# uberkk/ImageCompressionLearnedLiftingandLearnedTreeBasedModels

Hardware: AMD Instinct MI355X
Metric: Mpixels/sec (lifting DWT + entropy-model fwd) at 512x512 RGB (higher is better)
Workload: dtype f32 storage, f16x3 arithmetic (3 fp16 MFMA products per fp32 MAC, fp32 accumulate)

## Files before the change

### imagecompressionlearnedliftingandlearnedtreebasedmodels_amd/csrc/conv_f16x3.hip

```cpp
#include "common.h"
#include "split_f16.h"
#include "lifting_f16.h"
#include <string.h>
#include <type_traits>

namespace lldwt {

constexpr int F3_CK = 32;
constexpr int F3_TH = 8, F3_TW = 32;
constexpr int F3_IH = F3_TH + 2, F3_IW = F3_TW + 2, F3_NPX = F3_IH * F3_IW;
constexpr int F3_PITCH = F3_CK * 2 + 16;
constexpr int F3_PART = F3_NPX * F3_PITCH;
constexpr int F3_BUF = 2 * F3_PART;
constexpr int F3_LDS = 2 * F3_BUF + 64;
constexpr int F3_OCB = 128;
constexpr int F3_STEP_BYTES = 2048;
constexpr int F3_CHUNK_BYTES = 9 * 2 * F3_STEP_BYTES;
constexpr int F3_HDR = 256;
constexpr int F3_NTASK = F3_NPX * (F3_CK / 8);
constexpr int F3_R = (F3_NTASK + 255) / 256;

constexpr int F1_HDR = 2048;
constexpr int F1_CHUNK_BYTES = 2 * F3_STEP_BYTES;
constexpr int F1_NBLK = (F3_NPX + 31) / 32;
// ... 538 lines not shown
                if (u == 22) F3_FUSED_BLOCK(0, sdst)
                if (u == 26) F3_FUSED_BLOCK(1, sdst)
                if (u == 30) F3_FUSED_BLOCK(2, sdst)
            } else {
                if (u < F3_R) F3_TASK_LOAD(u, c1)
                if (u >= 24) F3_TASK_STORE((u - 24) >> 1, (u - 24) & 1, c1, sdst)
            }
            const half8 A_h = ah[st % 6], A_l = al[st % 6];
#pragma unroll
            for (int n = 0; n < 4; ++n) {
                if constexpr (PREC == 0) {
                    acc[hf * 4 + n] = mma32<0>(A_l, bh[u & 1][n], acc[hf * 4 + n]);
                    if constexpr (!IN16) acc[hf * 4 + n] = mma32<0>(A_h, bl[u & 1][n], acc[hf * 4 + n]);
                }
                acc[hf * 4 + n] = mma32<PREC>(A_h, bh[u & 1][n], acc[hf * 4 + n]);
            }
#pragma unroll
            for (int i = 0; i < (PREC == 0 ? 12 : 4); ++i) {
                __builtin_amdgcn_sched_group_barrier(0x008, 1, 0);
                __builtin_amdgcn_sched_group_barrier(0x100, 1, 0);
                __builtin_amdgcn_sched_group_barrier(0x020, 1, 0);
                __builtin_amdgcn_sched_group_barrier(0x002, PREC == 0 ? 4 : 10, 0);
                __builtin_amdgcn_sched_group_barrier(0x200, 1, 0);
            }
            __builtin_amdgcn_sched_barrier(0);
        }
#undef F3_BLOAD
        __syncthreads();
    }
    }
#undef F3_TASK_LOAD
#undef F3_TASK_STORE
#undef F3_FUSED_BLOCK
#undef F3_FUSED_LOAD

    F3_STAMP(10)
    if constexpr (S16) {
        const int px = lane & 15;
        const int ocw = ocb * F3_OCB + __builtin_amdgcn_readfirstlane(wave) * 32;
        const int och = 4 * (lane >> 4);
        float* ybase = a.y + (z * a.cout + ocw) * hw + (int64_t)y0 * w;
        const unsigned loff = (unsigned)och * (unsigned)hw + (unsigned)(x0 + px);
        const bool full = y0 + F3_TH <= h && x0 + F3_TW <= w;
        const float slope = a.act == LLDWT_ACT_LRELU ? 0.01f : (a.act == LLDWT_ACT_RELU ? 0.f : 1.f);
#pragma unroll
        for (int hv = 0; hv < 2; ++hv) {
#pragma unroll
            for (int q = 0; q < 4; ++q) {
                const int oc = ocw + 16 * hv + och + q;
                if (oc < a.cout) {
                    const float bq = a.bias ? a.bias[plane * a.cout + oc] : 0.f;
                    float* yq = ybase + (int64_t)(16 * hv + q) * hw;
                    if (full && a.act != LLDWT_ACT_TANH) {
#pragma unroll
                        for (int n = 0; n < 16; ++n) {
                            const float v = acc16[hv][n][q] * out_scale + bq;
                            yq[(n >> 1) * w + 16 * (n & 1) + loff] = fmaxf(v, v * slope);
                        }
                    } else {
#pragma unroll
                        for (int n = 0; n < 16; ++n)
                            if (y0 + (n >> 1) < h && x0 + 16 * (n & 1) + px < w)
                                yq[(n >> 1) * w + 16 * (n & 1) + loff] = act_apply(acc16[hv][n][q] * out_scale + bq, a.act);
                    }
                }
            }
        }
    } else {
        const int gx = x0 + (lane & 31);
        const int ocw = ocb * F3_OCB + __builtin_amdgcn_readfirstlane(wave) * 32;
        const int och = 4 * (lane >> 5);
        float* ybase = a.y + (z * a.cout + ocw) * hw + (int64_t)y0 * w;
        const unsigned loff = (unsigned)och * (unsigned)hw + (unsigned)gx;
        float bq[16];
#pragma unroll
        for (int q = 0; q < 16; ++q) {
            const int oc = ocw + (q & 3) + 8 * (q >> 2) + och;
            bq[q] = a.bias ? a.bias[plane * a.cout + (oc < a.cout ? oc : a.cout - 1)] : 0.f;
        }
#pragma unroll
        for (int q = 0; q < 16; ++q) asm volatile("" ::"v"(bq[q]));
        const bool full = y0 + F3_TH <= h && x0 + F3_TW <= w;
        if (full && a.act != LLDWT_ACT_TANH) {
            const float slope = a.act == LLDWT_ACT_LRELU ? 0.01f : (a.act == LLDWT_ACT_RELU ? 0.f : 1.f);
#pragma unroll
            for (int q = 0; q < 16; ++q) {
                if (ocw + (q & 3) + 8 * (q >> 2) + och < a.cout) {
                    float* yq = ybase + (int64_t)((q & 3) + 8 * (q >> 2)) * hw;
#pragma unroll
                    for (int n = 0; n < 8; ++n) {
                        const float v = acc[n][q] * out_scale + bq[q];
                        yq[n * w + loff] = fmaxf(v, v * slope);
                    }
                }
            }
        } else if (full) {
#pragma unroll
            for (int q = 0; q < 16; ++q) {
                if (ocw + (q & 3) + 8 * (q >> 2) + och < a.cout) {
                    float* yq = ybase + (int64_t)((q & 3) + 8 * (q >> 2)) * hw;
#pragma unroll
                    for (int n = 0; n < 8; ++n) yq[n * w + loff] = fast_tanh(acc[n][q] * out_scale + bq[q]);
                }
            }
        } else {
#pragma unroll
            for (int q = 0; q < 16; ++q) {
                if (ocw + (q & 3) + 8 * (q >> 2) + och < a.cout) {
                    float* yq = ybase + (int64_t)((q & 3) + 8 * (q >> 2)) * hw;
#pragma unroll
                    for (int n = 0; n < 8; ++n)
                        if (y0 + n < h && gx < w) yq[n * w + loff] = act_apply(acc[n][q] * out_scale + bq[q], a.act);
                }
            }
        }
    }
    F3_STAMP(11)
    F3_STAMP(15)
}

constexpr int W3_NE = F3_IH * 4 * 16;
constexpr int W3_PART = W3_NE * 32;
constexpr int W3_BUF = 2 * W3_PART;
constexpr int W3_DUMP = 2 * W3_BUF;
constexpr int W3_COLP = 144;
constexpr int W3_COL = W3_DUMP + 64;
constexpr int W3_PP = W3_COL + 2 * F3_IH * 17 * W3_COLP;
constexpr int W3_BIAS = W3_PP + 1536;
constexpr int W3_LDS = W3_BIAS + F3_OCB * 4;
constexpr int W3_LDS_EARLIER = W3_BIAS;
constexpr int W3_RING = 6;
static_assert(12 % W3_RING == 0 && W3_RING <= 6, "weight ring");
static_assert(W3_PP % 16 == 0 && F1_PP * 4 <= 1536, "LDS layout");

__device__ __forceinline__ void w3_row_mma(f4_t (&t)[4], const h8_t& wh, const h8_t& wl, const h8_t (&ch)[4], const h8_t (&cl)[4]) {
    asm volatile(
        "v_mfma_f32_16x16x32_f16 %0, %4, %6, 0\n\t"
        "v_mfma_f32_16x16x32_f16 %1, %4, %7, 0\n\t"
        "v_mfma_f32_16x16x32_f16 %2, %4, %8, 0\n\t"
        "v_mfma_f32_16x16x32_f16 %3, %4, %9, 0\n\t"
        "v_mfma_f32_16x16x32_f16 %0, %5, %10, %0\n\t"
        "v_mfma_f32_16x16x32_f16 %1, %5, %11, %1\n\t"
        "v_mfma_f32_16x16x32_f16 %2, %5, %12, %2\n\t"
        "v_mfma_f32_16x16x32_f16 %3, %5, %13, %3\n\t"
        "v_mfma_f32_16x16x32_f16 %0, %5, %6, %0\n\t"
        "v_mfma_f32_16x16x32_f16 %1, %5, %7, %1\n\t"
        "v_mfma_f32_16x16x32_f16 %2, %5, %8, %2\n\t"
        "v_mfma_f32_16x16x32_f16 %3, %5, %9, %3\n\t"
        "s_nop 7\n\ts_nop 7\n\ts_nop 4"
        : "=&v"(t[0]), "=&v"(t[1]), "=&v"(t[2]), "=&v"(t[3])
        : "v"(wl), "v"(wh), "v"(ch[0]), "v"(ch[1]), "v"(ch[2]), "v"(ch[3]), "v"(cl[0]), "v"(cl[1]), "v"(cl[2]), "v"(cl[3]));
}

__device__ __forceinline__ void wino_u(const float* g, double (&u)[4]) {
    const double g0 = g[0], g1 = g[1], g2 = g[2];
    u[0] = g0; u[1] = (g0 + g1 + g2) * 0.5; u[2] = (g0 - g1 + g2) * 0.5; u[3] = g2;
}

__global__ void k_f3w_umax(const float* __restrict__ w, int64_t nrows, uint8_t* __restrict__ packed, int64_t plane_bytes, int64_t woff) {
    const int plane = blockIdx.y;
    float m = 0.f;
    for (int64_t i = blockIdx.x * (int64_t)blockDim.x + threadIdx.x; i < nrows; i += (int64_t)gridDim.x * blockDim.x) {
        double u[4];
        wino_u(w + ((int64_t)plane * nrows + i) * 3, u);
        for (int k = 0; k < 4; ++k) m = fmaxf(m, fabsf((float)u[k]));
    }
#pragma unroll
    for (int o = 32; o > 0; o >>= 1) m = fmaxf(m, __shfl_down(m, o, 64));
    float* hdr = reinterpret_cast<float*>(packed + (int64_t)plane * plane_bytes + woff);
    if ((threadIdx.x & 63) == 0 && m > 0.f) atomicMax(reinterpret_cast<int*>(hdr + 1), __float_as_int(m));
}

__global__ void k_f3w_pack(const float* __restrict__ w, uint8_t* __restrict__ packed, int cin, int cout, int64_t plane_bytes, int64_t woff) {
    const int plane = blockIdx.y;
    uint8_t* pp = packed + (int64_t)plane * plane_bytes + woff;
    float* hdr = reinterpret_cast<float*>(pp);
    const double su = pow2_scale<15>(hdr[1]);
    const int nch = w3_nch(cin), nocb = (cout + F3_OCB - 1) / F3_OCB;
    const int64_t n = (int64_t)nocb * 4 * nch * W3_NST * 64 * 8;
    const float* wp = w + (int64_t)plane * cout * cin * 9;
    _Float16* out = reinterpret_cast<_Float16*>(pp + F3_HDR);
    for (int64_t i = blockIdx.x * (int64_t)blockDim.x + threadIdx.x; i < n; i += (int64_t)gridDim.x * blockDim.x) {
        int64_t r = i;
        const int j = (int)(r % 8); r /= 8;
        const int lane = (int)(r % 64); r /= 64;
        const int st = (int)(r % W3_NST); r /= W3_NST;
        const int chunk = (int)(r % nch); r /= nch;
        const int wv = (int)(r % 4); r /= 4;
        const int ocb = (int)r;
        const int oc = ocb * F3_OCB + wv * 32 + (lane & 31), ic = chunk * W3_CK + 8 * (lane >> 5) + j;
        const int dy = st >> 2, xi = st & 3;
        float v = 0.f;
        if (oc < cout && ic < cin) {
            double u[4];
            wino_u(wp + ((int64_t)oc * cin + ic) * 9 + dy * 3, u);
            v = (float)(u[xi] * su);
        }
        const _Float16 hi = (_Float16)v;
        const int64_t step = ((int64_t)(ocb * 4 + wv) * nch + chunk) * W3_NST + st;
        out[step * 1024 + lane * 8 + j] = hi;
        out[step * 1024 + 512 + lane * 8 + j] = (_Float16)(v - (float)hi);
    }
    if (blockIdx.x == 0 && threadIdx.x == 0) hdr[0] = (float)su;
}

template <bool EARLIER>
__global__ __launch_bounds__(256) __attribute__((amdgpu_waves_per_eu(1, 1))) void k_plc_wino(F3Args a) {
    extern __shared__ __attribute__((aligned(16))) uint8_t lds[];
    const int tid = threadIdx.x, lane = tid & 63, wave = tid >> 6;
    const int64_t z = blockIdx.z;
    const int plane = (int)(z / a.batch);
    const int ocb = blockIdx.y;
    const int ty = blockIdx.x / a.tiles_x, tx = blockIdx.x - ty * a.tiles_x;
    const int y0 = ty * F3_TH, x0 = tx * F3_TW;
    const int h = a.h, w = a.w;
    const int64_t hw = (int64_t)h * w;

    F3_STAMP(0)
    F3_STAMP(14)
    const uint8_t* pp = a.packed + (int64_t)plane * a.plane_bytes + f3_wino_off(a.cin, a.cout);
    const float su = *reinterpret_cast<const float*>(pp);
    const uint8_t* pk1 = a.packed1 + (int64_t)plane * a.plane_bytes1;
    const float* h1 = reinterpret_cast<const float*>(pk1);
    const float* bias1 = h1 + 16;
    const uint8_t* wbase = pp + F3_HDR + ((int64_t)(ocb * 4 + wave) * a.nch) * (W3_NST * F3_STEP_BYTES) + lane * 16;
    half8 ah[W3_RING], al[W3_RING];
#pragma unroll
    for (int i = 0; i < W3_RING - 1; ++i) {
        ah[i] = *reinterpret_cast<const half8*>(wbase + i * F3_STEP_BYTES);
        al[i] = *reinterpret_cast<const half8*>(wbase + i * F3_STEP_BYTES + 1024);
    }
    half8 w1h, w1l;
    f4_t b1r, b1v;
#define W3_FUSED_LOAD(C1)                                                                                             \
    {                                                                                                                 \
        const uint8_t* w1_ = pk1 + f1_w16_off(a.cin) + (int64_t)((C1) / W3_CK) * F3_STEP_BYTES + lane * 16;           \
        w1h = *reinterpret_cast<const half8*>(w1_);                                                                   \
        w1l = *reinterpret_cast<const half8*>(w1_ + 1024);                                                            \
        b1r = *reinterpret_cast<const f4_t*>(bias1 + (C1) + 4 * (lane >> 4));                                        \
    }
    W3_FUSED_LOAD(0)
    float bias2 = 0.f;
    if constexpr (!EARLIER) {
        const int oc = ocb * F3_OCB + tid;
        if (tid < F3_OCB && a.bias && oc < a.cout) bias2 = a.bias[plane * a.cout + oc];
    }

    const int hp = h >> 1, wp_ = w >> 1;
    const float* par = a.parent + z * 3 * (int64_t)hp * wp_;
    float* PP = reinterpret_cast<float*>(lds + W3_PP);
    float amax = 0.f;
#pragma unroll
    for (int i = tid; i < F1_PP; i += 256) {
        const int ci = i / 108, rem = i - ci * 108, r = rem / 18, c = rem - r * 18;
        const int Yp = (y0 >> 1) - 1 + r, Xp = (x0 >> 1) - 1 + c;
        const bool in = Yp >= 0 && Yp < hp && Xp >= 0 && Xp < wp_;
        const float v = par[(int64_t)ci * hp * wp_ + min(max(Yp, 0), hp - 1) * wp_ + min(max(Xp, 0), wp_ - 1)];
        const float vz = in ? v : 0.f;
        PP[i] = vz;
        amax = fmaxf(amax, fabsf(vz));
    }
#pragma unroll
    for (int o = 32; o > 0; o >>= 1) amax = fmaxf(amax, __shfl_xor(amax, o, 64));
    float* red = reinterpret_cast<float*>(lds + W3_DUMP + 32);
    if (lane == 0) red[wave] = amax;
    __syncthreads();
    amax = fmaxf(fmaxf(red[0], red[1]), fmaxf(red[2], red[3]));
    const float s_p = pow2_scale<15>(amax);
    const float sx = 0.5f * pow2_scale<15>(amax * h1[1] + h1[2]);
    const float out_scale = (1.f / sx) * (1.f / su);
    const float inv1sx = (1.f / s_p) * (1.f / h1[0]) * sx;
    for (int px = tid; px < F3_NPX; px += 256) {
        const int ly = px / F3_IW, lx = px - ly * F3_IW;
        uint8_t* dst = lds + W3_COL + ((lx & 1) * (F3_IH * 17) + ly * 17 + (lx >> 1)) * W3_COLP;
#pragma unroll
        for (int g = 0; g < 4; ++g) {
            float v8[8];
#pragma unroll
            for (int j = 0; j < 8; ++j) {
                const int k = 8 * g + j, q = k < 27 ? k : 26;
                const int dy = (q % 9) / 3, dx = q % 3;
                v8[j] = PP[(q / 9) * 108 + ((ly + dy) >> 1) * 18 + ((lx + dx) >> 1)] * s_p;
            }
            half8 ch_, cl_;
            split8v(v8, ch_, cl_);
            *reinterpret_cast<half8*>(dst + g * 16) = ch_;
            *reinterpret_cast<half8*>(dst + 64 + g * 16) = cl_;
        }
    }

    const int p = lane & 15, g = lane >> 4;
    int colw[3], vw[3];
    unsigned pinm = 0;
    bool pin[3][4];
#pragma unroll
    for (int B = 0; B < 3; ++B) {
        const int r = wave + 4 * B;
        const bool live = r < F3_IH;
        const int rr = live ? r : 0;
        colw[B] = W3_COL + (rr * 17 + p) * W3_COLP + g * 16;
        vw[B] = live ? ((rr * 4) * 16 + p) * 32 + (((g >> 1) ^ (p >> 3)) * 16) + (g & 1) * 8 : -1;
        const int gy = y0 - 1 + r;
#pragma unroll
        for (int s = 0; s < 4; ++s) {
            const int gx = x0 - 1 + 2 * p + s;
            pin[B][s] = live && gy >= 0 && gy < h && gx >= 0 && gx < w;
            if (pin[B][s]) pinm |= 1u << (4 * B + s);
        }
    }
    half8 c1h[4], c1l[4];
    f4_t t1[4];
    float d1[4][4];
#define W3_ROW_READ(B)                                                                                                \
    {                                                                                                                 \
        _Pragma("unroll") for (int s = 0; s < 4; ++s) {                                                               \
            const uint8_t* c_ = lds + colw[B] + ((s & 1) * (F3_IH * 17) + (s >> 1)) * W3_COLP;                        \
            c1h[s] = *reinterpret_cast<const half8*>(c_);                                                             \
            c1l[s] = *reinterpret_cast<const half8*>(c_ + 64);                                                        \
        }                                                                                                             \
    }
#define W3_ROW_MMA() w3_row_mma(t1, w1h, w1l, c1h, c1l);
#define W3_ROW_ACT(B)                                                                                                 \
    {                                                                                                                 \
        if ((B) == 0) b1v = b1r * sx;                                                                                 \
        _Pragma("unroll") for (int s = 0; s < 4; ++s)                                                                 \
            _Pragma("unroll") for (int q = 0; q < 4; ++q) {                                                           \
                const float v_ = __builtin_fmaf(t1[s][q], inv1sx, b1v[q]);                                            \
                d1[s][q] = (pinm >> (4 * (B) + s)) & 1 ? fmaxf(v_, 0.01f * v_) : 0.f;                                 \
            }                                                                                                         \
    }
#define W3_ROW_STORE(B, DST)                                                                                          \
    {                                                                                                                 \
        const bool livev_ = vw[B] >= 0;                                                                               \
        uint8_t* d0_ = livev_ ? (DST) + vw[B] : lds + W3_DUMP;                                                        \
        const int xs_ = livev_ ? 16 * 32 : 0, lo_ = livev_ ? W3_PART : 8;                                             \
        _Pragma("unroll") for (int xi = 0; xi < 4; ++xi) {                                                            \
            float v4_[4];                                                                                             \
            _Pragma("unroll") for (int q = 0; q < 4; ++q)                                                             \
                v4_[q] = xi == 0 ? d1[0][q] - d1[2][q] : xi == 1 ? d1[1][q] + d1[2][q]                                \
                       : xi == 2 ? d1[2][q] - d1[1][q] : d1[1][q] - d1[3][q];                                         \
            h4_t hi_, lo4_;                                                                                           \
            split4v(v4_, hi_, lo4_);                                                                                  \
            *reinterpret_cast<h4_t*>(d0_ + xi * xs_) = hi_;                                                           \
            *reinterpret_cast<h4_t*>(d0_ + xi * xs_ + lo_) = lo4_;                                                    \
        }                                                                                                             \
    }
    if constexpr (!EARLIER) {
        if (tid < F3_OCB) reinterpret_cast<float*>(lds + W3_BIAS)[tid] = bias2;
    }
#define W3_ROW_ACT1(B, S)                                                                                             \
    {                                                                                                                 \
        if ((B) == 0 && (S) == 0) b1v = b1r * sx;                                                                     \
        _Pragma("unroll") for (int q = 0; q < 4; ++q) {                                                               \
            const float v_ = __builtin_fmaf(t1[S][q], inv1sx, b1v[q]);                                                \
            d1[S][q] = pin[B][S] ? fmaxf(v_, 0.01f * v_) : 0.f;                                                       \
        }                                                                                                             \
    }
#define W3_ROW_STORE1(B, DST, XI)                                                                                     \
    {                                                                                                                 \
        const bool livev_ = vw[B] >= 0;                                                                               \
        uint8_t* d0_ = livev_ ? (DST) + vw[B] : lds + W3_DUMP;                                                        \
        const int xs_ = livev_ ? 16 * 32 : 0, lo_ = livev_ ? W3_PART : 8;                                             \
        float v4_[4];                                                                                                 \
        _Pragma("unroll") for (int q = 0; q < 4; ++q)                                                                 \
            v4_[q] = (XI) == 0 ? d1[0][q] - d1[2][q] : (XI) == 1 ? d1[1][q] + d1[2][q]                                \
                   : (XI) == 2 ? d1[2][q] - d1[1][q] : d1[1][q] - d1[3][q];                                           \
        h4_t hi_, lo4_;                                                                                               \
        split4v(v4_, hi_, lo4_);                                                                                      \
        *reinterpret_cast<h4_t*>(d0_ + (XI) * xs_) = hi_;                                                             \
        *reinterpret_cast<h4_t*>(d0_ + (XI) * xs_ + lo_) = lo4_;                                                      \
    }
    __syncthreads();

    floatx16 acc[4][4];
#pragma unroll
    for (int xi = 0; xi < 4; ++xi)
#pragma unroll
        for (int n = 0; n < 4; ++n)
#pragma unroll
            for (int q = 0; q < 16; ++q) acc[xi][n][q] = 0.f;

#pragma unroll
    for (int B = 0; B < 3; ++B) {
        W3_ROW_READ(B)
        W3_ROW_MMA()
        W3_ROW_ACT(B)
        W3_ROW_STORE(B, lds)
    }
    __syncthreads();

    const int boff = (((lane >> 4) & 1) * 64 + p) * 32 + (((lane >> 5) ^ (p >> 3)) * 16);
    F3_STAMP(1)
    for (int chunk = 0; chunk < a.nch; ++chunk) {
        if (chunk < 16 && !(chunk & 1)) F3_STAMP(2 + (chunk >> 1))
        const int buf = chunk & 1;
        const uint8_t* wp = wbase + (int64_t)chunk * (W3_NST * F3_STEP_BYTES);
        const uint8_t* bb = lds + buf * W3_BUF + boff;
        uint8_t* sdst = lds + (buf ^ 1) * W3_BUF;
        const int c1 = (chunk + 1 < a.nch ? chunk + 1 : chunk) * W3_CK;
        half8 bh[2][4], bl[2][4];
#define W3_BLOAD(U, SET)                                                                               \
        {                                                                                              \
            const int dy_ = (U) >> 2, xi_ = (U) & 3;                                                   \
            _Pragma("unroll") for (int n = 0; n < 4; ++n) {                                            \
                const int off = ((2 * n + dy_) * 4 + xi_) * 512;                                       \
                bh[SET][n] = *reinterpret_cast<const half8*>(bb + off);                                \
                bl[SET][n] = *reinterpret_cast<const half8*>(bb + W3_PART + off);                      \
            }                                                                                          \
        }
        W3_BLOAD(0, 0)
        __builtin_amdgcn_sched_barrier(0);
#pragma unroll
        for (int u = 0; u < W3_NST; ++u) {
            const int xi = u & 3;
            ah[(u + W3_RING - 1) % W3_RING] = *reinterpret_cast<const half8*>(wp + (u + W3_RING - 1) * F3_STEP_BYTES);
            al[(u + W3_RING - 1) % W3_RING] = *reinterpret_cast<const half8*>(wp + (u + W3_RING - 1) * F3_STEP_BYTES + 1024);
            if (u + 1 < W3_NST) W3_BLOAD(u + 1, (u + 1) & 1)
            if (u == 0) W3_FUSED_LOAD(c1)
            if constexpr (EARLIER) {
                if (u == 2 || u == 5 || u == 8) W3_ROW_READ((u - 2) / 3)
                if (u == 3 || u == 6 || u == 9) W3_ROW_MMA()
                if (u == 4 || u == 7 || u == 10) W3_ROW_ACT((u - 4) / 3)
                if (u == 5 || u == 8 || u == 11) W3_ROW_STORE((u - 5) / 3, sdst)
            } else {
                if (u == 2) W3_ROW_READ(0)
                if (u == 3) { W3_ROW_MMA() W3_ROW_READ(1) }
                if (u == 4) { W3_ROW_ACT1(0, 0) W3_ROW_ACT1(0, 2) W3_ROW_STORE1(0, sdst, 0) }
                if (u == 5) { W3_ROW_ACT1(0, 1) W3_ROW_STORE1(0, sdst, 1) W3_ROW_STORE1(0, sdst, 2) }
                if (u == 6) { W3_ROW_ACT1(0, 3) W3_ROW_STORE1(0, sdst, 3) W3_ROW_MMA() W3_ROW_READ(2) }
                if (u == 7) { W3_ROW_ACT1(1, 0) W3_ROW_ACT1(1, 2) W3_ROW_STORE1(1, sdst, 0) }
                if (u == 8) { W3_ROW_ACT1(1, 1) W3_ROW_ACT1(1, 3) W3_ROW_STORE1(1, sdst, 1) W3_ROW_MMA() }
                if (u == 9) { W3_ROW_STORE1(1, sdst, 2) W3_ROW_STORE1(1, sdst, 3) W3_ROW_ACT1(2, 0) }
                if (u == 10) { W3_ROW_ACT1(2, 2) W3_ROW_STORE1(2, sdst, 0) W3_ROW_ACT1(2, 1) }
                if (u == 11) { W3_ROW_STORE1(2, sdst, 1) W3_ROW_STORE1(2, sdst, 2) W3_ROW_ACT1(2, 3) W3_ROW_STORE1(2, sdst, 3) }
            }
            const half8 A_h = ah[u % W3_RING], A_l = al[u % W3_RING];
#pragma unroll
            for (int n = 0; n < 4; ++n) acc[xi][n] = mma32<0>(A_l, bh[u & 1][n], acc[xi][n]);
#pragma unroll
            for (int n = 0; n < 4; ++n) acc[xi][n] = mma32<0>(A_h, bl[u & 1][n], acc[xi][n]);
#pragma unroll
            for (int n = 0; n < 4; ++n) acc[xi][n] = mma32<0>(A_h, bh[u & 1][n], acc[xi][n]);
#pragma unroll
            for (int i = 0; i < 12; ++i) {
                __builtin_amdgcn_sched_group_barrier(0x008, 1, 0);
                __builtin_amdgcn_sched_group_barrier(0x100, 1, 0);
                __builtin_amdgcn_sched_group_barrier(0x020, 1, 0);
                if constexpr (EARLIER) __builtin_amdgcn_sched_group_barrier(0x002, 8, 0);
                else if (u == 11 || i >= 8) __builtin_amdgcn_sched_group_barrier(0x002, 6, 0);
                else __builtin_amdgcn_sched_group_barrier(0x002, 4, 0);
                __builtin_amdgcn_sched_group_barrier(0x200, 1, 0);
            }
            __builtin_amdgcn_sched_barrier(0);
        }
#undef W3_BLOAD
        __syncthreads();
    }
#undef W3_ROW_READ
#undef W3_ROW_MMA
#undef W3_ROW_ACT
#undef W3_ROW_STORE
#undef W3_ROW_ACT1
#undef W3_ROW_STORE1
#undef W3_FUSED_LOAD

    F3_STAMP(10)
    const int ocw = ocb * F3_OCB + __builtin_amdgcn_readfirstlane(wave) * 32;
    const int och = 4 * (lane >> 5), orow = (lane >> 4) & 1;
    float* ybase = a.y + (z * a.cout + ocw) * hw + (int64_t)y0 * w;
    const unsigned loff = (unsigned)och * (unsigned)hw + (unsigned)(orow * w + x0 + 2 * p);
    const bool full = y0 + F3_TH <= h && x0 + F3_TW <= w;
    if constexpr (EARLIER) {
#define W3_EPI(COND, ACT0, ACT1)                                                                                      \
    _Pragma("unroll") for (int q = 0; q < 16; ++q) {                                                                  \
        const int ocq = (q & 3) + 8 * (q >> 2);                                                                       \
        if (ocw + ocq + och < a.cout) {                                                                               \
            const float bq = a.bias ? a.bias[plane * a.cout + ocw + ocq + och] : 0.f;                                 \
            float* yq = ybase + (int64_t)ocq * hw + loff;                                                             \
            _Pragma("unroll") for (int n = 0; n < 4; ++n) {                                                           \
                const float v0 = (acc[0][n][q] + acc[1][n][q] + acc[2][n][q]) * out_scale + bq;                       \
                const float v1 = (acc[1][n][q] - acc[2][n][q] - acc[3][n][q]) * out_scale + bq;                       \
                if (COND) *reinterpret_cast<f2_t*>(yq + 2 * n * w) = f2_t{ACT0, ACT1};                                \
            }                                                                                                         \
        }                                                                                                             \
    }
    if (full && a.act != LLDWT_ACT_TANH) {
        const float slope = a.act == LLDWT_ACT_LRELU ? 0.01f : (a.act == LLDWT_ACT_RELU ? 0.f : 1.f);
        W3_EPI(true, fmaxf(v0, v0 * slope), fmaxf(v1, v1 * slope))
    } else {
        const bool colin = x0 + 2 * p < w;
        W3_EPI(colin && y0 + 2 * n + orow < h, act_apply(v0, a.act), act_apply(v1, a.act))
    }
#undef W3_EPI
    } else {
    float bq[16];
    {
        const f4_t* bl = reinterpret_cast<const f4_t*>(lds + W3_BIAS + (__builtin_amdgcn_readfirstlane(wave) * 32 + och) * 4);
#pragma unroll
        for (int k = 0; k < 4; ++k) {
            const f4_t b4 = bl[2 * k];
#pragma unroll
            for (int j = 0; j < 4; ++j) bq[4 * k + j] = b4[j];
        }
    }
#define W3_EPI(COND, ACT0, ACT1)                                                                                      \
    _Pragma("unroll") for (int q = 0; q < 16; ++q) {                                                                  \
        const int ocq = (q & 3) + 8 * (q >> 2);                                                                       \
        if (ocw + ocq + och < a.cout) {                                                                               \
            float* yq = ybase + (int64_t)ocq * hw + loff;                                                             \
            _Pragma("unroll") for (int n = 0; n < 4; ++n) {                                                           \
                const float v0 = (acc[0][n][q] + acc[1][n][q] + acc[2][n][q]) * out_scale + bq[q];                    \
                const float v1 = (acc[1][n][q] - acc[2][n][q] - acc[3][n][q]) * out_scale + bq[q];                    \
                if (COND) *reinterpret_cast<f2_t*>(yq + 2 * n * w) = f2_t{ACT0, ACT1};                                \
            }                                                                                                         \
        }                                                                                                             \
    }
    if (full && a.act != LLDWT_ACT_TANH) {
        const float slope = a.act == LLDWT_ACT_LRELU ? 0.01f : (a.act == LLDWT_ACT_RELU ? 0.f : 1.f);
        W3_EPI(true, fmaxf(v0, v0 * slope), fmaxf(v1, v1 * slope))
    } else {
        const bool colin = x0 + 2 * p < w;
#define W3_IN (colin && y0 + 2 * n + orow < h)
        if (a.act == LLDWT_ACT_TANH) {
            W3_EPI(W3_IN, fast_tanh(v0), fast_tanh(v1))
        } else if (a.act == LLDWT_ACT_LRELU) {
            W3_EPI(W3_IN, v0 >= 0.f ? v0 : 0.01f * v0, v1 >= 0.f ? v1 : 0.01f * v1)
        } else if (a.act == LLDWT_ACT_RELU) {
            W3_EPI(W3_IN, v0 > 0.f ? v0 : 0.f, v1 > 0.f ? v1 : 0.f)
        } else {
            W3_EPI(W3_IN, v0, v1)
        }
#undef W3_IN
    }
#undef W3_EPI
    }
    F3_STAMP(11)
    F3_STAMP(15)
}
#undef F3_STAMP

}
using namespace lldwt;

static const int g_f3_shape16 = [] { const char* e = getenv("LLDWT_PLC_SHAPE"); return (e && !strcmp(e, "16")) ? 1 : 0; }();
static int f3_shape16() { return g_f3_shape16; }
extern "C" int lldwt_plc_shape16(void) { return g_f3_shape16; }

static const int g_plc_wino = [] { const char* e = getenv("LLDWT_PLC_ALGO"); return (e && !strcmp(e, "direct")) ? 0 : 1; }();
static bool plc_wino_active() { return g_plc_wino && !g_f3_shape16; }
extern "C" int lldwt_plc_winograd(void) { return plc_wino_active() ? 1 : 0; }

extern "C" int64_t lldwt_conv_f16x3_packed_bytes(int cin, int cout) {
    if (cin <= 0 || cout <= 0) return -1;
    return f3_plane_bytes(cin, cout);
}

extern "C" int lldwt_conv_f16x3_pack(const float* w, void* packed, int cin, int cout, int64_t planes, void* stream) {
    LLDWT_REQUIRE(w && packed && cin > 0 && cout > 0 && planes > 0 && planes <= 65535, "conv_f16x3_pack: bad arguments");
    hipStream_t st = (hipStream_t)stream;
    const int64_t pb = f3_plane_bytes(cin, cout);
    for (int64_t p = 0; p < planes; ++p)
        if (hipMemsetAsync(reinterpret_cast<char*>(packed) + p * pb, 0, F3_HDR, st) != hipSuccess) {
            set_error("conv_f16x3_pack: memset failed");
            return LLDWT_EHIP;
        }
    const int64_t nw = (int64_t)cout * cin * 9;
    hipLaunchKernelGGL(k_f3_wmax, dim3(64, (unsigned)planes), dim3(256), 0, st, w, nw, reinterpret_cast<float*>(packed), pb);
    hipLaunchKernelGGL(k_f3_pack, dim3(1024, (unsigned)planes), dim3(256), 0, st, w, reinterpret_cast<uint8_t*>(packed), cin, cout, pb,
                       f3_shape16());
    if (plc_wino_active()) {
        const int64_t wo = f3_wino_off(cin, cout);
        for (int64_t p = 0; p < planes; ++p)
            if (hipMemsetAsync(reinterpret_cast<char*>(packed) + p * pb + wo, 0, F3_HDR, st) != hipSuccess) {
                set_error("conv_f16x3_pack: memset failed");
                return LLDWT_EHIP;
            }
        hipLaunchKernelGGL(k_f3w_umax, dim3(64, (unsigned)planes), dim3(256), 0, st, w, (int64_t)cout * cin * 3,
                           reinterpret_cast<uint8_t*>(packed), pb, wo);
        hipLaunchKernelGGL(k_f3w_pack, dim3(1024, (unsigned)planes), dim3(256), 0, st, w, reinterpret_cast<uint8_t*>(packed), cin, cout,
                           pb, wo);
    }
    return check_launch("conv_f16x3_pack");
}

extern "C" int lldwt_absmax_slots(const float* x, int64_t planes, int64_t n_per_plane, float* slots, void* stream) {
    LLDWT_REQUIRE(x && slots && planes > 0 && planes <= 65535 && n_per_plane > 0, "absmax_slots: bad arguments");
    const int vec = (((uintptr_t)x) & 15) == 0 && (n_per_plane & 3) == 0;
    hipStream_t st = (hipStream_t)stream;
    if (hipMemsetAsync(slots, 0, sizeof(float) * 64 * planes, st) != hipSuccess) {
        set_error("absmax_slots: memset failed");
        return LLDWT_EHIP;
    }
    int64_t gx = cdiv(n_per_plane / 4 + 1, 256 * 8);
    gx = gx < 1 ? 1 : (gx > 2048 ? 2048 : gx);
    hipLaunchKernelGGL(k_absmax_slots, dim3((unsigned)gx, (unsigned)planes), dim3(256), 0, st, x, n_per_plane, slots, vec);
    return check_launch("absmax_slots");
}

extern "C" int lldwt_conv3x3_f16x3(const float* x, float* y, const void* packed, const float* bias, const float* slots,
                                   int cin, int cout, int act, int64_t planes, int64_t batch, int64_t h, int64_t w_,
                                   void* stream) {
    LLDWT_REQUIRE(x && y && packed && slots, "conv3x3_f16x3: null pointer");
    LLDWT_REQUIRE(cin > 0 && cout > 0 && planes > 0 && batch > 0 && h > 0 && w_ > 0 && planes * batch <= 65535,
                  "conv3x3_f16x3: bad dims");
    LLDWT_REQUIRE(act == LLDWT_ACT_NONE || act == LLDWT_ACT_LRELU || act == LLDWT_ACT_TANH || act == LLDWT_ACT_RELU, "conv3x3_f16x3: bad activation");
    LLDWT_REQUIRE((int64_t)F3_CK * h * w_ * 4 < (int64_t)1 << 32, "conv3x3_f16x3: image too large for 32-bit chunk offsets");
    F3Args a;
    a.x = x; a.y = y; a.packed = reinterpret_cast<const uint8_t*>(packed); a.bias = bias; a.slots = slots;
    a.x16 = nullptr; a.xscale = nullptr; a.parent = nullptr; a.packed1 = nullptr; a.plane_bytes1 = 0; a.stamps = nullptr;
    a.cin = cin; a.cout = cout; a.act = act; a.batch = (int)batch; a.h = (int)h; a.w = (int)w_;
    a.tiles_x = (int)cdiv(w_, F3_TW);
    a.nch = f3_nch(cin);
    a.plane_bytes = f3_plane_bytes(cin, cout);
    const int tiles_y = (int)cdiv(h, F3_TH);
    static bool attr_set = false;
    if (!attr_set) {
// ... 120 lines not shown
```

Measured before the change: 207.5.

## Restructure fused lifting conv pipeline with DPP halo sharing and earlier sync

In the non-EARLIER path, the first-stage row MMA now computes two column phases plus one extra edge column per row. The other two phases are rebuilt with DPP cross-lane shifts instead of extra MFMAs, which cuts the first-stage MFMA count. The per-chunk schedule changes too: B-operand loads for the next chunk are prefetched before the barrier, the barrier moves to the second-to-last step, and the fused weight load runs two chunks ahead. The im2col fill is split so each wave handles one channel group, and a hand-written split4 replaces split4v. This adds register pressure and subtle halo and boundary logic that could break correctness at tile edges.

After: 211.4, median of 6. 1.9% higher.

```diff
diff --git a/imagecompressionlearnedliftingandlearnedtreebasedmodels_amd/csrc/conv_f16x3.hip b/imagecompressionlearnedliftingandlearnedtreebasedmodels_amd/csrc/conv_f16x3.hip
--- a/imagecompressionlearnedliftingandlearnedtreebasedmodels_amd/csrc/conv_f16x3.hip
+++ b/imagecompressionlearnedliftingandlearnedtreebasedmodels_amd/csrc/conv_f16x3.hip
@@ -714,6 +714,63 @@
         : "v"(wl), "v"(wh), "v"(ch[0]), "v"(ch[1]), "v"(ch[2]), "v"(ch[3]), "v"(cl[0]), "v"(cl[1]), "v"(cl[2]), "v"(cl[3]));
 }
 
+__device__ __forceinline__ void w3_row_mma2(f4_t& t0, f4_t& t1, const h8_t& wh, const h8_t& wl, const h8_t& ch0, const h8_t& ch1,
+                                            const h8_t& cl0, const h8_t& cl1) {
+    asm volatile(
+        "v_mfma_f32_16x16x32_f16 %0, %2, %4, 0\n\t"
+        "v_mfma_f32_16x16x32_f16 %1, %2, %5, 0\n\t"
+        "v_mfma_f32_16x16x32_f16 %0, %3, %6, %0\n\t"
+        "v_mfma_f32_16x16x32_f16 %1, %3, %7, %1\n\t"
+        "v_mfma_f32_16x16x32_f16 %0, %3, %4, %0\n\t"
+        "v_mfma_f32_16x16x32_f16 %1, %3, %5, %1\n\t"
+        "s_nop 7\n\ts_nop 7\n\ts_nop 4"
+        : "=&v"(t0), "=&v"(t1)
+        : "v"(wl), "v"(wh), "v"(ch0), "v"(ch1), "v"(cl0), "v"(cl1));
+}
+__device__ __forceinline__ void w3_row_mma3(f4_t& t0, f4_t& t1, f4_t& t2, const h8_t& wh, const h8_t& wl, const h8_t& ch0,
+                                            const h8_t& ch1, const h8_t& ch2, const h8_t& cl0, const h8_t& cl1, const h8_t& cl2) {
+    asm volatile(
+        "v_mfma_f32_16x16x32_f16 %0, %3, %5, 0\n\t"
+        "v_mfma_f32_16x16x32_f16 %1, %3, %6, 0\n\t"
+        "v_mfma_f32_16x16x32_f16 %2, %3, %7, 0\n\t"
+        "v_mfma_f32_16x16x32_f16 %0, %4, %8, %0\n\t"
+        "v_mfma_f32_16x16x32_f16 %1, %4, %9, %1\n\t"
+        "v_mfma_f32_16x16x32_f16 %2, %4, %10, %2\n\t"
+        "v_mfma_f32_16x16x32_f16 %0, %4, %5, %0\n\t"
+        "v_mfma_f32_16x16x32_f16 %1, %4, %6, %1\n\t"
+        "v_mfma_f32_16x16x32_f16 %2, %4, %7, %2\n\t"
+        "s_nop 7\n\ts_nop 7\n\ts_nop 4"
+        : "=&v"(t0), "=&v"(t1), "=&v"(t2)
+        : "v"(wl), "v"(wh), "v"(ch0), "v"(ch1), "v"(ch2), "v"(cl0), "v"(cl1), "v"(cl2));
+}
+template <int CTRL, bool BOUND>
+__device__ __forceinline__ float w3_dpp(float old, float src) {
+    return __int_as_float(__builtin_amdgcn_update_dpp(__float_as_int(old), __float_as_int(src), CTRL, 0xf, 0xf, BOUND));
+}
+__device__ __forceinline__ void w3_split4(const float (&v)[4], h4_t& hi, h4_t& lo) {
+    const f4_t x = {v[0], v[1], v[2], v[3]};
+    hi = __builtin_convertvector(x, h4_t);
+    lo = __builtin_convertvector(x - __builtin_convertvector(hi, f4_t), h4_t);
+}
+template <int G>
+__device__ __forceinline__ void w3_im2col_group(uint8_t* lds, const float* PP, float s_p, int lane) {
+    for (int px = lane; px < F3_NPX; px += 64) {
+        const int ly = px / F3_IW, lx = px - ly * F3_IW;
+        uint8_t* dst = lds + W3_COL + ((lx & 1) * (F3_IH * 17) + ly * 17 + (lx >> 1)) * W3_COLP;
+        float v8[8];
+#pragma unroll
+        for (int j = 0; j < 8; ++j) {
+            const int k = 8 * G + j, q = k < 27 ? k : 26;
+            const int dy = (q % 9) / 3, dx = q % 3;
+            v8[j] = PP[(q / 9) * 108 + ((ly + dy) >> 1) * 18 + ((lx + dx) >> 1)] * s_p;
+        }
+        half8 ch_, cl_;
+        split8v(v8, ch_, cl_);
+        *reinterpret_cast<half8*>(dst + G * 16) = ch_;
+        *reinterpret_cast<half8*>(dst + 64 + G * 16) = cl_;
+    }
+}
+
 __device__ __forceinline__ void wino_u(const float* g, double (&u)[4]) {
     const double g0 = g[0], g1 = g[1], g2 = g[2];
     u[0] = g0; u[1] = (g0 + g1 + g2) * 0.5; u[2] = (g0 - g1 + g2) * 0.5; u[3] = g2;
@@ -832,6 +889,8 @@
     const float sx = 0.5f * pow2_scale<15>(amax * h1[1] + h1[2]);
     const float out_scale = (1.f / sx) * (1.f / su);
     const float inv1sx = (1.f / s_p) * (1.f / h1[0]) * sx;
+    F3_STAMP(12)
+    if constexpr (EARLIER) {
     for (int px = tid; px < F3_NPX; px += 256) {
         const int ly = px / F3_IW, lx = px - ly * F3_IW;
         uint8_t* dst = lds + W3_COL + ((lx & 1) * (F3_IH * 17) + ly * 17 + (lx >> 1)) * W3_COLP;
@@ -848,6 +907,14 @@
             split8v(v8, ch_, cl_);
             *reinterpret_cast<half8*>(dst + g * 16) = ch_;
             *reinterpret_cast<half8*>(dst + 64 + g * 16) = cl_;
+        }
+    }
+    } else {
+        switch (__builtin_amdgcn_readfirstlane(wave)) {
+            case 0: w3_im2col_group<0>(lds, PP, s_p, lane); break;
+            case 1: w3_im2col_group<1>(lds, PP, s_p, lane); break;
+            case 2: w3_im2col_group<2>(lds, PP, s_p, lane); break;
+            default: w3_im2col_group<3>(lds, PP, s_p, lane); break;
         }
     }
 
@@ -870,6 +937,10 @@
             if (pin[B][s]) pinm |= 1u << (4 * B + s);
         }
     }
+    const int en = p < 6 ? p : 0, er = wave + 4 * (en >> 1);
+    const bool elive = p < 6 && er < F3_IH;
+    const int cole = W3_COL + (((en & 1) * F3_IH + (elive ? er : 0)) * 17 + 16) * W3_COLP + g * 16;
+    const int pine = (elive && y0 - 1 + er >= 0 && y0 - 1 + er < h && x0 + 31 + (en & 1) < w) ? -1 : 0;
     half8 c1h[4], c1l[4];
     f4_t t1[4];
     float d1[4][4];
@@ -910,91 +981,142 @@
     if constexpr (!EARLIER) {
         if (tid < F3_OCB) reinterpret_cast<float*>(lds + W3_BIAS)[tid] = bias2;
     }
-#define W3_ROW_ACT1(B, S)                                                                                             \
+    half8 c2h[3][2], c2l[3][2], ceh, cel;
+    f4_t t2[3][2], te;
+    float d2[3][4][4], de[4];
+#define W3_ROW_READ2(B)                                                                                               \
     {                                                                                                                 \
-        if ((B) == 0 && (S) == 0) b1v = b1r * sx;                                                                     \
+        _Pragma("unroll") for (int s = 0; s < 2; ++s) {                                                               \
+            const uint8_t* c_ = lds + colw[B] + s * (F3_IH * 17) * W3_COLP;                                           \
+            c2h[B][s] = *reinterpret_cast<const half8*>(c_);                                                          \
+            c2l[B][s] = *reinterpret_cast<const half8*>(c_ + 64);                                                     \
+        }                                                                                                             \
+    }
+#define W3_ROW_MMA2(B) w3_row_mma2(t2[B][0], t2[B][1], w1h, w1l, c2h[B][0], c2h[B][1], c2l[B][0], c2l[B][1]);
+#define W3_ROW_MMA3() w3_row_mma3(t2[0][0], t2[0][1], te, w1h, w1l, c2h[0][0], c2h[0][1], ceh, c2l[0][0], c2l[0][1], cel);
+#define W3_ROW_ACT2(B, S)                                                                                             \
+    {                                                                                                                 \
         _Pragma("unroll") for (int q = 0; q < 4; ++q) {                                                               \
-            const float v_ = __builtin_fmaf(t1[S][q], inv1sx, b1v[q]);                                                \
-            d1[S][q] = pin[B][S] ? fmaxf(v_, 0.01f * v_) : 0.f;                                                       \
+            const float v_ = __builtin_fmaf(t2[B][S][q], inv1sx, b1v[q]);                                             \
+            d2[B][S][q] = pin[B][S] ? fmaxf(v_, 0.01f * v_) : 0.f;                                                    \
         }                                                                                                             \
     }
-#define W3_ROW_STORE1(B, DST, XI)                                                                                     \
+#define W3_EXTRA_ACT()                                                                                                \
+    {                                                                                                                 \
+        b1v = b1r * sx;                                                                                               \
+        _Pragma("unroll") for (int q = 0; q < 4; ++q) {                                                               \
+            const float v_ = __builtin_fmaf(te[q], inv1sx, b1v[q]);                                                   \
+            de[q] = __int_as_float(__float_as_int(fmaxf(v_, 0.01f * v_)) & pine);                                     \
+        }                                                                                                             \
+    }
+#define W3_ROW_SHIFT(B)                                                                                               \
+    {                                                                                                                 \
+        _Pragma("unroll") for (int q = 0; q < 4; ++q) {                                                               \
+            d2[B][2][q] = w3_dpp<0x101, false>(w3_dpp<0x110 + 15 - 2 * (B), true>(0.f, de[q]), d2[B][0][q]);          \
+            d2[B][3][q] = w3_dpp<0x101, false>(w3_dpp<0x110 + 14 - 2 * (B), true>(0.f, de[q]), d2[B][1][q]);          \
+        }                                                                                                             \
+    }
+#define W3_ROW_STORE2(B, DST, XI)                                                                                     \
     {                                                                                                                 \
         const bool livev_ = vw[B] >= 0;                                                                               \
         uint8_t* d0_ = livev_ ? (DST) + vw[B] : lds + W3_DUMP;                                                        \
         const int xs_ = livev_ ? 16 * 32 : 0, lo_ = livev_ ? W3_PART : 8;                                             \
         float v4_[4];                                                                                                 \
         _Pragma("unroll") for (int q = 0; q < 4; ++q)                                                                 \
-            v4_[q] = (XI) == 0 ? d1[0][q] - d1[2][q] : (XI) == 1 ? d1[1][q] + d1[2][q]                                \
-                   : (XI) == 2 ? d1[2][q] - d1[1][q] : d1[1][q] - d1[3][q];                                           \
+            v4_[q] = (XI) == 0 ? d2[B][0][q] - d2[B][2][q] : (XI) == 1 ? d2[B][1][q] + d2[B][2][q]                    \
+                   : (XI) == 2 ? d2[B][2][q] - d2[B][1][q] : d2[B][1][q] - d2[B][3][q];                               \
         h4_t hi_, lo4_;                                                                                               \
-        split4v(v4_, hi_, lo4_);                                                                                      \
+        w3_split4(v4_, hi_, lo4_);                                                                                    \
         *reinterpret_cast<h4_t*>(d0_ + (XI) * xs_) = hi_;                                                             \
         *reinterpret_cast<h4_t*>(d0_ + (XI) * xs_ + lo_) = lo4_;                                                      \
     }
+    F3_STAMP(13)
     __syncthreads();
+    F3_STAMP(2)
 
     floatx16 acc[4][4];
-#pragma unroll
-    for (int xi = 0; xi < 4; ++xi)
-#pragma unroll
-        for (int n = 0; n < 4; ++n)
-#pragma unroll
-            for (int q = 0; q < 16; ++q) acc[xi][n][q] = 0.f;
-
-#pragma unroll
-    for (int B = 0; B < 3; ++B) {
-        W3_ROW_READ(B)
-        W3_ROW_MMA()
-        W3_ROW_ACT(B)
-        W3_ROW_STORE(B, lds)
-    }
+#define W3_ZERO_ACC()                                                                                                 \
+    _Pragma("unroll") for (int xi = 0; xi < 4; ++xi)                                                                  \
+        _Pragma("unroll") for (int n = 0; n < 4; ++n)                                                                 \
+            _Pragma("unroll") for (int q = 0; q < 16; ++q) acc[xi][n][q] = 0.f;
+    if constexpr (EARLIER) {
+        W3_ZERO_ACC()
+#pragma unroll
+        for (int B = 0; B < 3; ++B) {
+            W3_ROW_READ(B)
+            W3_ROW_MMA()
+            W3_ROW_ACT(B)
+            W3_ROW_STORE(B, lds)
+        }
+    } else {
+        ceh = *reinterpret_cast<const half8*>(lds + cole);
+        cel = *reinterpret_cast<const half8*>(lds + cole + 64);
+        W3_ROW_READ2(0) W3_ROW_READ2(1) W3_ROW_READ2(2)
+        W3_ROW_MMA3() W3_ROW_MMA2(1) W3_ROW_MMA2(2)
+        W3_EXTRA_ACT()
+        W3_FUSED_LOAD((a.nch > 1 ? 1 : 0) * W3_CK)
+        W3_ROW_ACT2(0, 0) W3_ROW_ACT2(0, 1) W3_ROW_SHIFT(0)
+        W3_ROW_STORE2(0, lds, 0) W3_ROW_STORE2(0, lds, 1) W3_ROW_STORE2(0, lds, 2) W3_ROW_STORE2(0, lds, 3)
+        W3_ROW_ACT2(1, 0) W3_ROW_ACT2(1, 1) W3_ROW_SHIFT(1)
+        W3_ROW_STORE2(1, lds, 0) W3_ROW_STORE2(1, lds, 1) W3_ROW_STORE2(1, lds, 2) W3_ROW_STORE2(1, lds, 3)
+        W3_ROW_ACT2(2, 0) W3_ROW_ACT2(2, 1) W3_ROW_SHIFT(2)
+        W3_ROW_STORE2(2, lds, 0) W3_ROW_STORE2(2, lds, 1) W3_ROW_STORE2(2, lds, 2) W3_ROW_STORE2(2, lds, 3)
+        W3_ZERO_ACC()
+    }
+#undef W3_ZERO_ACC
     __syncthreads();
 
     const int boff = (((lane >> 4) & 1) * 64 + p) * 32 + (((lane >> 5) ^ (p >> 3)) * 16);
+    half8 bh[2][4], bl[2][4];
+#define W3_BLOAD_AT(BB, U, SET)                                                                        \
+        {                                                                                              \
+            const int dy_ = (U) >> 2, xi_ = (U) & 3;                                                   \
+            _Pragma("unroll") for (int n = 0; n < 4; ++n) {                                            \
+                const int off = ((2 * n + dy_) * 4 + xi_) * 512;                                       \
+                bh[SET][n] = *reinterpret_cast<const half8*>((BB) + off);                              \
+                bl[SET][n] = *reinterpret_cast<const half8*>((BB) + W3_PART + off);                    \
+            }                                                                                          \
+        }
+    if constexpr (!EARLIER) W3_BLOAD_AT(lds + boff, 0, 0)
     F3_STAMP(1)
     for (int chunk = 0; chunk < a.nch; ++chunk) {
-        if (chunk < 16 && !(chunk & 1)) F3_STAMP(2 + (chunk >> 1))
+        if (chunk >= 2 && chunk < 16 && !(chunk & 1)) F3_STAMP(2 + (chunk >> 1))
         const int buf = chunk & 1;
         const uint8_t* wp = wbase + (int64_t)chunk * (W3_NST * F3_STEP_BYTES);
         const uint8_t* bb = lds + buf * W3_BUF + boff;
         uint8_t* sdst = lds + (buf ^ 1) * W3_BUF;
         const int c1 = (chunk + 1 < a.nch ? chunk + 1 : chunk) * W3_CK;
-        half8 bh[2][4], bl[2][4];
-#define W3_BLOAD(U, SET)                                                                               \
-        {                                                                                              \
-            const int dy_ = (U) >> 2, xi_ = (U) & 3;                                                   \
-            _Pragma("unroll") for (int n = 0; n < 4; ++n) {                                            \
-                const int off = ((2 * n + dy_) * 4 + xi_) * 512;                                       \
-                bh[SET][n] = *reinterpret_cast<const half8*>(bb + off);                                \
-                bl[SET][n] = *reinterpret_cast<const half8*>(bb + W3_PART + off);                      \
-            }                                                                                          \
-        }
-        W3_BLOAD(0, 0)
-        __builtin_amdgcn_sched_barrier(0);
+        const int c2 = (chunk + 2 < a.nch ? chunk + 2 : a.nch - 1) * W3_CK;
+#define W3_BLOAD(U, SET) W3_BLOAD_AT(bb, U, SET)
+        if constexpr (EARLIER) {
+            W3_BLOAD(0, 0)
+            __builtin_amdgcn_sched_barrier(0);
+        }
 #pragma unroll
         for (int u = 0; u < W3_NST; ++u) {
             const int xi = u & 3;
             ah[(u + W3_RING - 1) % W3_RING] = *reinterpret_cast<const half8*>(wp + (u + W3_RING - 1) * F3_STEP_BYTES);
             al[(u + W3_RING - 1) % W3_RING] = *reinterpret_cast<const half8*>(wp + (u + W3_RING - 1) * F3_STEP_BYTES + 1024);
             if (u + 1 < W3_NST) W3_BLOAD(u + 1, (u + 1) & 1)
-            if (u == 0) W3_FUSED_LOAD(c1)
             if constexpr (EARLIER) {
+                if (u == 0) W3_FUSED_LOAD(c1)
                 if (u == 2 || u == 5 || u == 8) W3_ROW_READ((u - 2) / 3)
                 if (u == 3 || u == 6 || u == 9) W3_ROW_MMA()
                 if (u == 4 || u == 7 || u == 10) W3_ROW_ACT((u - 4) / 3)
                 if (u == 5 || u == 8 || u == 11) W3_ROW_STORE((u - 5) / 3, sdst)
             } else {
-                if (u == 2) W3_ROW_READ(0)
-                if (u == 3) { W3_ROW_MMA() W3_ROW_READ(1) }
-                if (u == 4) { W3_ROW_ACT1(0, 0) W3_ROW_ACT1(0, 2) W3_ROW_STORE1(0, sdst, 0) }
-                if (u == 5) { W3_ROW_ACT1(0, 1) W3_ROW_STORE1(0, sdst, 1) W3_ROW_STORE1(0, sdst, 2) }
-                if (u == 6) { W3_ROW_ACT1(0, 3) W3_ROW_STORE1(0, sdst, 3) W3_ROW_MMA() W3_ROW_READ(2) }
-                if (u == 7) { W3_ROW_ACT1(1, 0) W3_ROW_ACT1(1, 2) W3_ROW_STORE1(1, sdst, 0) }
-                if (u == 8) { W3_ROW_ACT1(1, 1) W3_ROW_ACT1(1, 3) W3_ROW_STORE1(1, sdst, 1) W3_ROW_MMA() }
-                if (u == 9) { W3_ROW_STORE1(1, sdst, 2) W3_ROW_STORE1(1, sdst, 3) W3_ROW_ACT1(2, 0) }
-                if (u == 10) { W3_ROW_ACT1(2, 2) W3_ROW_STORE1(2, sdst, 0) W3_ROW_ACT1(2, 1) }
-                if (u == 11) { W3_ROW_STORE1(2, sdst, 1) W3_ROW_STORE1(2, sdst, 2) W3_ROW_ACT1(2, 3) W3_ROW_STORE1(2, sdst, 3) }
+                if (u == W3_NST - 1) W3_BLOAD_AT(sdst + boff, 0, 0)
+                if (u == 0) W3_ROW_READ2(0)
+                if (u == 1) { W3_ROW_MMA3() W3_ROW_READ2(1) }
+                if (u == 2) { W3_EXTRA_ACT() W3_ROW_ACT2(0, 0) W3_ROW_ACT2(0, 1) W3_ROW_MMA2(1) W3_ROW_READ2(2) }
+                if (u == 3) { W3_ROW_SHIFT(0) W3_ROW_STORE2(0, sdst, 0) W3_ROW_STORE2(0, sdst, 1) }
+                if (u == 4) { W3_ROW_STORE2(0, sdst, 2) W3_ROW_STORE2(0, sdst, 3) W3_ROW_ACT2(1, 0) W3_ROW_MMA2(2) }
+                if (u == 5) { W3_ROW_ACT2(1, 1) W3_ROW_SHIFT(1) W3_ROW_STORE2(1, sdst, 0) }
+                if (u == 6) { W3_ROW_STORE2(1, sdst, 1) W3_ROW_STORE2(1, sdst, 2) W3_ROW_ACT2(2, 0) }
+                if (u == 7) { W3_ROW_STORE2(1, sdst, 3) W3_ROW_ACT2(2, 1) W3_ROW_SHIFT(2) }
+                if (u == 8) { W3_ROW_STORE2(2, sdst, 0) W3_ROW_STORE2(2, sdst, 1) W3_FUSED_LOAD(c2) }
+                if (u == 9) W3_ROW_STORE2(2, sdst, 2)
+                if (u == 10) W3_ROW_STORE2(2, sdst, 3)
             }
             const half8 A_h = ah[u % W3_RING], A_l = al[u % W3_RING];
 #pragma unroll
@@ -1009,21 +1131,30 @@
                 __builtin_amdgcn_sched_group_barrier(0x100, 1, 0);
                 __builtin_amdgcn_sched_group_barrier(0x020, 1, 0);
                 if constexpr (EARLIER) __builtin_amdgcn_sched_group_barrier(0x002, 8, 0);
-                else if (u == 11 || i >= 8) __builtin_amdgcn_sched_group_barrier(0x002, 6, 0);
+                else if (i >= 8) __builtin_amdgcn_sched_group_barrier(0x002, 6, 0);
                 else __builtin_amdgcn_sched_group_barrier(0x002, 4, 0);
                 __builtin_amdgcn_sched_group_barrier(0x200, 1, 0);
             }
             __builtin_amdgcn_sched_barrier(0);
+            if constexpr (!EARLIER) {
+                if (u == W3_NST - 2) __syncthreads();
+            }
         }
 #undef W3_BLOAD
-        __syncthreads();
-    }
+        if constexpr (EARLIER) __syncthreads();
+    }
+#undef W3_BLOAD_AT
 #undef W3_ROW_READ
 #undef W3_ROW_MMA
 #undef W3_ROW_ACT
 #undef W3_ROW_STORE
-#undef W3_ROW_ACT1
-#undef W3_ROW_STORE1
+#undef W3_ROW_READ2
+#undef W3_ROW_MMA2
+#undef W3_ROW_MMA3
+#undef W3_ROW_ACT2
+#undef W3_EXTRA_ACT
+#undef W3_ROW_SHIFT
+#undef W3_ROW_STORE2
 #undef W3_FUSED_LOAD
 
     F3_STAMP(10)
```
